# lauraset/Super-resolution-building-height-estimation

Hardware: AMD Instinct MI355X
Metric: tiles/sec (64x64x8ch->256x256 height) (higher is better)
Workload: dtype f16 operands / f32 accumulate (MFMA), f32 residual stream; 1 GPU; RRDBNet x4 (23 RRDB, 64 feat) forward_feature, batch 32 tiles/GPU, 64x64x3 -> 64x256x256 (BASELINE.json configs[1]); global_batch=32, parallelism=tile-sharded x1 (no data-path collective)

## Files before the change

include/srbh.h:

```cpp
#ifndef SRBH_H
#define SRBH_H

#include <stddef.h>
#include <stdint.h>

#ifdef __cplusplus
extern "C" {
#endif

#define SRBH_OK 0
#define SRBH_ERR_ARG (-1)
#define SRBH_ERR_WORKSPACE (-2)

int srbh_version(void);
const char* srbh_last_error(void);
#define SRBH_PATH_HCONV16 0
#define SRBH_PATH_HCONV_TEMPLATE 1
#define SRBH_PATH_ENTRY_FUSED 2
#define SRBH_PATH_ENTRY_SPLIT 3
#define SRBH_PATH_WGRAD16 4
#define SRBH_PATH_WGRAD_B16_GENERIC 5
#define SRBH_PATH_WGRAD_F32 6
#define SRBH_PATH_WGRAD_ENTRY_FUSED 7
#define SRBH_PATH_WGRAD_ENTRY_SPLIT 8
#define SRBH_PATH_HCONV_UP 9
#define SRBH_PATH_HBLOCK16 11
#define SRBH_PATH_HBWD16 10
int srbh_path_counters(unsigned long long* out, int n, int reset);
int srbh_head_wgs_cap(int path);

size_t srbh_act16_bytes(int B, int C, int H, int W);
int srbh_nchw32_to_act16(const float* src, void* dst, int B, int C, int H, int W, void* stream);
int srbh_act16_to_nchw32(const void* src, float* dst, int B, int C, int H, int W, void* stream);

size_t srbh_wpack16_bytes(int cout, int cin);
int srbh_pack_conv3x3_f16(const float* w_oihw, int cout, int cin, void* packed, void* stream);

typedef struct srbh_conv3x3_args {
    const void* in;
    int in_chunks_total;
    int in_chunk0;
    int in_chunks;
    const void* w;
    const float* bias;
    int cout;
    int B, H, W;
    int upsample2x;
    int lrelu;
    float res_scale;
    float* res1;
    int res1_update;
    float res2_scale;
    float* res2;
    int res2_update;
    const float* skip;
    void* out16;
    int out16_chunks_total;
    int out16_chunk0;
    float* out32;
    int out32_c;
    int out16_nhwc;
} srbh_conv3x3_args;

int srbh_conv3x3_f16(const srbh_conv3x3_args* a, void* stream);

typedef struct srbh_conv3x3_split {
    const void* in_lo;
    int in_lo_chunks_total;
    int in_lo_chunk0;
    const void* w_lo;
    void* out16_lo;
    int out16_lo_chunks_total;
    int out16_lo_chunk0;
} srbh_conv3x3_split;
int srbh_conv3x3_f16x2(const srbh_conv3x3_args* a, const srbh_conv3x3_split* s, void* stream);
int srbh_pack_conv3x3_f16lo(const float* w_oihw, int cout, int cin, void* packed, void* stream);
int srbh_act16_split_lo(const float* v, int fragment_order, const void* hi, int hi_chunks_total, int hi_chunk0, void* lo, int lo_chunks_total,
                        int lo_chunk0, int B, int H, int W, void* stream);
int srbh_conv3x3_x16(const srbh_conv3x3_args* a, int bf16, const void* mask16, int mask_chunks_total, int mask_chunk0, void* stream);
int srbh_pack_conv3x3_b16(const float* w_oihw, int cout, int cin, void* packed, void* stream);
typedef struct srbh_pack3x3_desc {
    const float* w;
    void* packed;
    const float* bias_src;
    float* bias_dst;
    int cout, cin, bf16, pad_;
} srbh_pack3x3_desc;
int srbh_pack_conv3x3_many(const srbh_pack3x3_desc* table_dev, int n, long max_elems, void* stream);
int srbh_nhwc32_to_act16(const float* src, void* dst, int B, int C, int H, int W, int chunks_total, int chunk0, float scale, int bf16,
                         void* stream);
int srbh_act16_channel_sum(const void* src, int B, int H, int W, int chunks_total, int chunk0, int nchunk, int bf16, float* out,
                           void* stream);
int srbh_act16_wgrad_b16(const void* x, int x_chunks_total, int cin, const void* dy, int dy_chunks_total, int dy_ch0, int cout,
                         int B, int H, int W, float* dw, float* ws, void* stream);
int srbh_axpby_f32(float* dst, float a, const float* x, float b, const float* y, long n, void* stream);
int srbh_lrelu_bwd_f32(float* g, const float* y, float slope, long n, void* stream);
int srbh_up2_bwd_nhwc_f32(const float* g, float* out, int B, int Ho, int Wo, int C, void* stream);
int srbh_bilinear2x_nhwc_f32(const float* x, float* out, int B, int H, int W, int C, int backward, void* stream);

int srbh_conv_first_f32(const float* x_nchw, const float* w_oihw, const float* bias, int B, int cin, int H, int W,
                        float* res_a, float* res_b, float* res_c, void* out16, int out16_chunks_total, void* stream);

typedef struct srbh_conv_w {
    const void* w;
    const float* bias;
} srbh_conv_w;

typedef struct srbh_rrdbnet_desc {
    int num_in_ch;
    int num_block;
    const float* conv_first_w;
    const float* conv_first_b;
    const srbh_conv_w* rdb;
    srbh_conv_w conv_body, conv_up1, conv_up2, conv_hr;
    srbh_conv_w conv_last;
    int num_out_ch;
    const srbh_conv_w* rdb_b16;
    int tail_f16x2;
    const void* conv_body_lo;
    const void* conv_up1_lo;
    const void* conv_up2_lo;
    const void* conv_hr_lo;
} srbh_rrdbnet_desc;

size_t srbh_rrdbnet_workspace_bytes(int B, int H, int W, int want_forward);
size_t srbh_rrdbnet_workspace_bytes_f16x2(int B, int H, int W, int want_forward);
int srbh_rrdbnet_forward(const srbh_rrdbnet_desc* d, const float* x, float* out, int B, int H, int W,
                         int want_forward, void* ws, size_t ws_bytes, void* stream);


int srbh_rrdbnet_trunk_train_forward(const srbh_rrdbnet_desc* d, float* xr, float* xrr, void* dense_all, size_t dense_stride, int B, int H,
                                     int W, void* stream);
size_t srbh_rrdbnet_trunk_train_aux_bytes(int B, int H, int W);
int srbh_rrdbnet_trunk_train_forward_persistent(const srbh_rrdbnet_desc* d, float* xr, float* xrr, void* dense_all, size_t dense_stride, int B, int H,
                                                int W, void* aux, void* stream, int* used);
size_t srbh_rrdbnet_trunk_wgrad_ws_bytes(void);
int srbh_rrdbnet_trunk_train_backward(int num_block, const void* dense_all, size_t dense_stride, const void* packs, size_t pack_stride,
                                      const size_t* pack_off, float* g_a, float* g_b, float* g_c, float** g_out, void* G, size_t g_stride,
                                      float* dw_all, float* db_all, float* wgrad_ws, int B, int H, int W, void* stream);
int srbh_rrdbnet_trunk_train_backward_persistent(int num_block, const void* dense_all, size_t dense_stride, const void* packs, size_t pack_stride,
                                                 const size_t* pack_off, const float* zero_bias, const float* g_a, float* g_b, float* g_c,
                                                 float** g_out, void* G_all, size_t g_stride, float* dw_all, float* db_all, float* wgrad_ws,
                                                 void* trunk_wgrad_ws, int B, int H, int W, void* aux, void* stream, int* used);
size_t srbh_trunk_wgrad_ws_bytes(int num_block, int B, int H, int W);
int srbh_trunk_wgrad(int num_block, const void* dense_all, size_t dense_stride, const void* G_all, size_t g_stride, int B, int H, int W, float* dw_all,
                     float* db_all, void* ws, void* stream);

int srbh_rrdbnet_last_status(const void* ws, int B, int H, int W, int want_forward, void* stream);

int srbh_rrdbnet_trunk_out(const void* ws, size_t ws_bytes, int num_block, int B, int H, int W, int want_forward, float* out, void* stream);

int srbh_ptail_wgs_cap(int cap);

int srbh_trunk_timing(int on);
int srbh_trunk_last_ms(float* ms);
const char* srbh_trunk_kernel_name(void);

size_t srbh_hpack_bytes(int cout, int cin, int ksize);
int srbh_hpack_conv_f32(const float* w_oihw, int cout, int cin, int ksize, int transpose_flip, float* packed, void* stream);

size_t srbh_bn_stats_bytes(int C);
int srbh_hconv_up_supported(int H, int W);

typedef struct srbh_hconv_args {
    const float* src0; int c0;
    const float* pre_scale; const float* pre_shift; int pre_relu;
    const float* src1; int c1;
    const float* w;
    const float* bias;
    int cout;
    int ksize;
    int B, H, W;
    int pixelshuffle2;
    float* out;
    double* stats;
    int src0_ld, src1_ld;
    int out_ld, out_coff;
    int post_lrelu;
    const float* res1; int res1_ld; float res1_scale;
    const float* res2; int res2_ld; float res2_scale;
// ... 278 lines not shown
```

super-resolution-building-height-estimation_amd/_lib.py:

```python
from __future__ import annotations

import ctypes as C
import os
import subprocess
import threading

_HERE = os.path.dirname(os.path.abspath(__file__))
ROOT = os.path.dirname(_HERE)
CSRC = os.path.join(_HERE, "csrc")
INCLUDE = os.path.join(ROOT, "include")
LIB_PATH = os.path.join(_HERE, "libsrbh.so")
_DEV_LIB = os.environ.get("SRBH_LIB_PATH")
SOURCES = ["srbh_conv3x3.hip", "srbh_aux.hip", "srbh_rrdbnet.hip", "srbh_ptrunk.hip", "srbh_trunk_wgrad.hip", "srbh_ptail.hip", "srbh_ptail_split.hip", "srbh_head.hip", "srbh_head_bwd.hip", "srbh_mosaic.hip", "srbh_loader.hip", "srbh_loss.hip", "srbh_dwconv.hip", "srbh_mbconv.hip", "srbh_pwconv.hip", "srbh_dconv.hip", "srbh_optim.hip"]
HIPCC = os.environ.get("HIPCC", "/opt/rocm/bin/hipcc")
HIPFLAGS = ["--offload-arch=gfx950", "-O3", "-std=c++17", "-fPIC", "-Wno-unused-result", "-Wno-inline-asm"]
if os.environ.get("SRBH_HIPFLAGS_OVERRIDE"):
    HIPFLAGS = os.environ["SRBH_HIPFLAGS_OVERRIDE"].split()


def build(force: bool = False, verbose: bool = False) -> str:
    srcs = [os.path.join(CSRC, s) for s in SOURCES if os.path.exists(os.path.join(CSRC, s))]
    deps = srcs + [os.path.join(CSRC, f) for f in os.listdir(CSRC) if f.endswith(".h")] + [os.path.join(INCLUDE, "srbh.h")]
    if not force and os.path.exists(LIB_PATH) and all(os.path.getmtime(LIB_PATH) >= os.path.getmtime(d) for d in deps):
        return LIB_PATH
    objs, procs = [], []
    for s in srcs:
        o = s[:-4] + ".o"
        objs.append(o)
        cmd = [HIPCC, *HIPFLAGS, "-I", INCLUDE, "-I", CSRC, "-c", s, "-o", o]
        procs.append((cmd, subprocess.Popen(cmd, stdout=subprocess.PIPE, stderr=subprocess.STDOUT, text=True)))
    for cmd, p in procs:
        out, _ = p.communicate()
        if p.returncode != 0:
            raise RuntimeError("hipcc failed: %s\n%s" % (" ".join(cmd), out))
        if verbose and out:
            print(out)
    cmd = [HIPCC, "--offload-arch=gfx950", "-shared", "-fPIC", *objs, "-o", LIB_PATH]
    r = subprocess.run(cmd, stdout=subprocess.PIPE, stderr=subprocess.STDOUT, text=True)
    if r.returncode != 0:
        raise RuntimeError("link failed: %s\n%s" % (" ".join(cmd), r.stdout))
    return LIB_PATH


PATH_NAMES = ("hconv16", "hconv_template", "entry_fused", "entry_split", "wgrad16", "wgrad_b16_generic", "wgrad_f32", "wgrad_entry_fused",
              "wgrad_entry_split", "hconv_up", "hbwd16", "hblock16")


def path_counters(reset=False):
    buf = (C.c_ulonglong * len(PATH_NAMES))()
    lib().srbh_path_counters(buf, len(PATH_NAMES), int(reset))
    return {k: int(v) for k, v in zip(PATH_NAMES, buf)}


def head_wgs_cap(form):
    cap = lib().srbh_head_wgs_cap(PATH_NAMES.index(form))
    if cap < 0:
        raise ValueError(f"{form}: no persistent tile walk behind this form")
    return int(cap)


class ConvArgs(C.Structure):
    _fields_ = [
        ("in_", C.c_void_p), ("in_chunks_total", C.c_int), ("in_chunk0", C.c_int), ("in_chunks", C.c_int),
        ("w", C.c_void_p), ("bias", C.c_void_p), ("cout", C.c_int),
        ("B", C.c_int), ("H", C.c_int), ("W", C.c_int),
        ("upsample2x", C.c_int), ("lrelu", C.c_int),
        ("res_scale", C.c_float), ("res1", C.c_void_p), ("res1_update", C.c_int),
        ("res2_scale", C.c_float), ("res2", C.c_void_p), ("res2_update", C.c_int),
        ("skip", C.c_void_p),
        ("out16", C.c_void_p), ("out16_chunks_total", C.c_int), ("out16_chunk0", C.c_int),
        ("out32", C.c_void_p), ("out32_c", C.c_int), ("out16_nhwc", C.c_int),
    ]


class HConvArgs(C.Structure):
    _fields_ = [
        ("src0", C.c_void_p), ("c0", C.c_int),
        ("pre_scale", C.c_void_p), ("pre_shift", C.c_void_p), ("pre_relu", C.c_int),
        ("src1", C.c_void_p), ("c1", C.c_int),
        ("w", C.c_void_p), ("bias", C.c_void_p), ("cout", C.c_int), ("ksize", C.c_int),
        ("B", C.c_int), ("H", C.c_int), ("W", C.c_int), ("pixelshuffle2", C.c_int),
        ("out", C.c_void_p), ("stats", C.c_void_p),
        ("src0_ld", C.c_int), ("src1_ld", C.c_int), ("out_ld", C.c_int), ("out_coff", C.c_int), ("post_lrelu", C.c_int),
        ("res1", C.c_void_p), ("res1_ld", C.c_int), ("res1_scale", C.c_float),
        ("res2", C.c_void_p), ("res2_ld", C.c_int), ("res2_scale", C.c_float),
        ("post_scale", C.c_void_p), ("post_shift", C.c_void_p), ("post_relu", C.c_int),
        ("io_h16", C.c_int),
        ("bstat_c", C.c_void_p), ("bstat_mean", C.c_void_p), ("bstat_invstd", C.c_void_p), ("bstat_ms", C.c_void_p), ("bstat_mh", C.c_void_p),
        ("stats_clean", C.c_int),
    ]


class HBwd16Args(C.Structure):
    _fields_ = ([("g", C.c_void_p), ("c", C.c_void_p), ("mean", C.c_void_p), ("invstd", C.c_void_p), ("coef", C.c_void_p), ("k1", C.c_void_p),
                 ("k2", C.c_void_p), ("mask_scale", C.c_void_p), ("mask_shift", C.c_void_p), ("x", C.c_void_p), ("pre_scale", C.c_void_p),
                 ("pre_shift", C.c_void_p), ("pre_relu", C.c_int), ("w", C.c_void_p), ("B", C.c_int), ("H", C.c_int), ("W", C.c_int),
                 ("dx", C.c_void_p), ("dx_b16", C.c_int), ("res", C.c_void_p), ("bstat_c", C.c_void_p), ("bstat_mean", C.c_void_p),
                 ("bstat_invstd", C.c_void_p), ("bstat_ms", C.c_void_p), ("bstat_mh", C.c_void_p), ("stats", C.c_void_p), ("stats_clean", C.c_int),
                 ("dw", C.c_void_p), ("ws", C.c_void_p), ("relu_bits", C.c_void_p)])


class HBlock16Args(C.Structure):
    _fields_ = [("x", C.c_void_p), ("w1", C.c_void_p), ("w2", C.c_void_p), ("scale1", C.c_void_p), ("shift1", C.c_void_p),
                ("scale2", C.c_void_p), ("shift2", C.c_void_p), ("out", C.c_void_p), ("out_h16", C.c_int), ("B", C.c_int), ("H", C.c_int), ("W", C.c_int)]


class HWGradArgs(C.Structure):
    _fields_ = [
        ("src0", C.c_void_p), ("c0", C.c_int),
        ("pre_scale", C.c_void_p), ("pre_shift", C.c_void_p), ("pre_relu", C.c_int),
        ("src1", C.c_void_p), ("c1", C.c_int),
        ("dy", C.c_void_p), ("cout", C.c_int), ("ksize", C.c_int),
        ("B", C.c_int), ("H", C.c_int), ("W", C.c_int), ("dw", C.c_void_p), ("ws", C.c_void_p),
        ("src0_ld", C.c_int), ("src1_ld", C.c_int), ("io", C.c_int),
    ]


class BnActArgs(C.Structure):
    _fields_ = [
        ("x", C.c_void_p), ("y", C.c_void_p), ("gamma", C.c_void_p), ("beta", C.c_void_p),
        ("running_mean", C.c_void_p), ("running_var", C.c_void_p), ("save_mean", C.c_void_p), ("save_invstd", C.c_void_p),
        ("pooled", C.c_void_p), ("res", C.c_void_p), ("drop", C.c_void_p),
        ("momentum", C.c_float), ("eps", C.c_float), ("B", C.c_int), ("C", C.c_int), ("HW", C.c_int), ("act", C.c_int),
        ("ws", C.c_void_p),
    ]


class MbMidArgs(C.Structure):
    _fields_ = ([(n, C.c_void_p) for n in ("e_pre", "wdw", "gamma0", "beta0", "running_mean0", "running_var0", "mean0", "invstd0",
                                           "gamma1", "beta1", "running_mean1", "running_var1", "mean1", "invstd1", "d_pre", "y", "pooled")]
                + [(n, C.c_float) for n in ("momentum0", "eps0", "momentum1", "eps1")] + [(n, C.c_int) for n in ("B", "C", "H", "W", "K")])


class MbMidBwdArgs(C.Structure):
    _fields_ = ([(n, C.c_void_p) for n in ("dout", "gate", "dpooled", "d_pre", "e_pre", "wdw", "gamma0", "beta0", "mean0", "invstd0",
                                           "gamma1", "beta1", "mean1", "invstd1", "de_pre", "dwdw", "dgamma0", "dbeta0", "dgamma1", "dbeta1")]
                + [(n, C.c_int) for n in ("B", "C", "H", "W", "K")])


class BnActBwdArgs(C.Structure):
    _fields_ = [
        ("dy", C.c_void_p), ("x", C.c_void_p), ("gamma", C.c_void_p), ("beta", C.c_void_p),
        ("save_mean", C.c_void_p), ("save_invstd", C.c_void_p), ("gate", C.c_void_p), ("dpooled", C.c_void_p), ("drop", C.c_void_p),
        ("dx", C.c_void_p), ("dgamma", C.c_void_p), ("dbeta", C.c_void_p),
        ("B", C.c_int), ("C", C.c_int), ("HW", C.c_int), ("act", C.c_int), ("ws", C.c_void_p),
    ]


class ConvW(C.Structure):
    _fields_ = [("w", C.c_void_p), ("bias", C.c_void_p)]


class RRDBNetDesc(C.Structure):
    _fields_ = [
        ("num_in_ch", C.c_int), ("num_block", C.c_int),
        ("conv_first_w", C.c_void_p), ("conv_first_b", C.c_void_p),
        ("rdb", C.POINTER(ConvW)),
        ("conv_body", ConvW), ("conv_up1", ConvW), ("conv_up2", ConvW), ("conv_hr", ConvW),
        ("conv_last", ConvW), ("num_out_ch", C.c_int),
        ("rdb_b16", C.POINTER(ConvW)),
        ("tail_f16x2", C.c_int),
        ("conv_body_lo", C.c_void_p), ("conv_up1_lo", C.c_void_p), ("conv_up2_lo", C.c_void_p), ("conv_hr_lo", C.c_void_p),
    ]


class ConvSplit(C.Structure):
    _fields_ = [
        ("in_lo", C.c_void_p), ("in_lo_chunks_total", C.c_int), ("in_lo_chunk0", C.c_int),
        ("w_lo", C.c_void_p),
        ("out16_lo", C.c_void_p), ("out16_lo_chunks_total", C.c_int), ("out16_lo_chunk0", C.c_int),
    ]


_vp, _i, _sz, _f = C.c_void_p, C.c_int, C.c_size_t, C.c_float
SIGNATURES = {
    "srbh_version": (_i, []),
    "srbh_last_error": (C.c_char_p, []),
    "srbh_path_counters": (_i, [_vp, _i, _i]),
    "srbh_head_wgs_cap": (_i, [_i]),
    "srbh_act16_bytes": (_sz, [_i, _i, _i, _i]),
    "srbh_nchw32_to_act16": (_i, [_vp, _vp, _i, _i, _i, _i, _vp]),
    "srbh_act16_to_nchw32": (_i, [_vp, _vp, _i, _i, _i, _i, _vp]),
    "srbh_wpack16_bytes": (_sz, [_i, _i]),
    "srbh_pack_conv3x3_f16": (_i, [_vp, _i, _i, _vp, _vp]),
    "srbh_conv3x3_f16": (_i, [C.POINTER(ConvArgs), _vp]),
    "srbh_conv3x3_f16x2": (_i, [C.POINTER(ConvArgs), C.POINTER(ConvSplit), _vp]),
    "srbh_pack_conv3x3_f16lo": (_i, [_vp, _i, _i, _vp, _vp]),
    "srbh_act16_split_lo": (_i, [_vp, _i, _vp, _i, _i, _vp, _i, _i, _i, _i, _i, _vp]),
    "srbh_rrdbnet_workspace_bytes_f16x2": (_sz, [_i, _i, _i, _i]),
    "srbh_conv3x3_x16": (_i, [C.POINTER(ConvArgs), _i, _vp, _i, _i, _vp]),
    "srbh_pack_conv3x3_b16": (_i, [_vp, _i, _i, _vp, _vp]),
    "srbh_nhwc32_to_act16": (_i, [_vp, _vp, _i, _i, _i, _i, _i, _i, _f, _i, _vp]),
    "srbh_act16_channel_sum": (_i, [_vp, _i, _i, _i, _i, _i, _i, _i, _vp, _vp]),
    "srbh_axpby_f32": (_i, [_vp, _f, _vp, _f, _vp, C.c_long, _vp]),
    "srbh_rrdbnet_trunk_train_forward": (_i, [C.POINTER(RRDBNetDesc), _vp, _vp, _vp, _sz, _i, _i, _i, _vp]),
    "srbh_rrdbnet_trunk_train_aux_bytes": (_sz, [_i, _i, _i]),
    "srbh_rrdbnet_trunk_train_forward_persistent": (_i, [C.POINTER(RRDBNetDesc), _vp, _vp, _vp, _sz, _i, _i, _i, _vp, _vp, C.POINTER(C.c_int)]),
    "srbh_rrdbnet_trunk_wgrad_ws_bytes": (_sz, []),
# ... 165 lines not shown
```

super-resolution-building-height-estimation_amd/csrc/srbh_internal.h:

```cpp
#pragma once
#include <hip/hip_runtime.h>
#include <stdarg.h>
#include <stdio.h>
#include <vector>
#include "srbh.h"

namespace srbh {

constexpr int PIX_B = 64;
constexpr int CHUNK_C = 32;
constexpr int TILE_W = 64;
constexpr int TILE_H = 8;

void set_error(const char* fmt, ...);
enum PathCounter { PATH_HCONV16 = 0, PATH_HCONV_TEMPLATE, PATH_ENTRY_FUSED, PATH_ENTRY_SPLIT, PATH_WGRAD16, PATH_WGRAD_B16_GENERIC,
                   PATH_WGRAD_F32, PATH_WGRAD_ENTRY_FUSED, PATH_WGRAD_ENTRY_SPLIT, PATH_HCONV_UP, PATH_HBWD16, PATH_HBLOCK16, PATH_N };
extern unsigned long long g_path_counters[PATH_N];
inline void count_path(int i) { ++g_path_counters[i]; }
int hconv16_wgs_cap();
int hconv_up_wgs_cap();
int hconv_entry_wgs_cap();
int hblock16_wgs_cap();
int hwgrad16_wgs_cap();
int hbwd16_wgs_cap();
int zero_async(void* p, size_t bytes, hipStream_t st);
int hip_fail(hipError_t e, const char* what);

#define SRBH_HIP(call)                                         \
    do {                                                       \
        hipError_t e_ = (call);                                \
        if (e_ != hipSuccess) return srbh::hip_fail(e_, #call); \
    } while (0)

#define SRBH_REQUIRE(cond, ...)            \
    do {                                   \
        if (!(cond)) {                     \
            srbh::set_error(__VA_ARGS__);  \
            return SRBH_ERR_ARG;           \
        }                                  \
    } while (0)

#define SRBH_ONCE_PER_DEVICE(stmt)                        \
    do {                                                  \
        static unsigned long long done_ = 0;              \
        int dev_ = 0;                                     \
        SRBH_HIP(hipGetDevice(&dev_));                    \
        if (!((done_ >> (dev_ & 63)) & 1ull)) {           \
            stmt;                                         \
            done_ |= 1ull << (dev_ & 63);                 \
        }                                                 \
    } while (0)

struct Act16Geo {
    int row_b;
    int plane_b;
    long img_b;
    size_t total_b;
};
inline Act16Geo act16_geo(int B, int chunks, int H, int W) {
    Act16Geo g;
    g.row_b = (W + 2) * PIX_B;
    g.plane_b = (H + 2) * g.row_b;
    g.img_b = (long)chunks * g.plane_b;
    size_t slack = (size_t)(TILE_H + 4) * (size_t)((W + 2 > TILE_W + 2) ? (W + 2) : (TILE_W + 2)) * PIX_B + 8192;
    g.total_b = (size_t)B * g.img_b + slack;
    g.total_b = (g.total_b + 255) & ~(size_t)255;
    return g;
}


size_t ptrunk_aux_bytes(int B, int tiles_per_img);
size_t ptrunk_err_offset(int B, int tiles_per_img);
int ptail_run(const srbh_conv3x3_args* a, hipStream_t stream, int* used);
int ptail_wgs_cap();
int ptrunk_takes(int num_block, int H, int W, int* takes, int* ncu_out);
int ptrunk_run(const srbh_rrdbnet_desc* d, void* dense0, void* dense1, float* xr, float* xrr, int B, int H, int W,
               void* aux, hipStream_t stream, int* used, int* final_cur, long train_stride = 0, const void* mask = nullptr, long mask_stride = 0,
               bool bf16 = false);
int conv3x3_trunk_b16(const srbh_conv3x3_args* a, int out_f16, void* stream);
int conv_first_f32(const float* x, const float* w, const float* bias, int B, int cin, int H, int W, float* ra, float* rb, float* rc,
                   void* out16, int out16_chunks_total, int bf16, void* stream);


#if defined(__HIP_DEVICE_COMPILE__) || defined(__HIPCC__)
__device__ __forceinline__ void fold_stat_slots(double* stats, const int C, const int clear, double* red, double& s, double& q) {
    constexpr int NS = 64;
    const int t = threadIdx.x, V = 2 * C, G = 256 / V, v = t % V, g = t / V;
    double part = 0.0;
    if (g < G) {
        for (int k = g; k < NS; k += G) part += stats[(long)k * V + v];
        if (clear)
            for (int k = g; k < NS; k += G) stats[(long)k * V + v] = 0.0;
        red[g * V + v] = part;
    }
    __syncthreads();
    s = 0.0;
    q = 0.0;
    if (t < C)
        for (int k = 0; k < G; ++k) {
            s += red[k * V + t];
            q += red[k * V + C + t];
        }
}

__device__ __forceinline__ unsigned bf16x2_rne(float lo, float hi) {
    typedef float f2_t __attribute__((ext_vector_type(2)));
    typedef __bf16 b2_t __attribute__((ext_vector_type(2)));
    const f2_t f = {lo, hi};
    return __builtin_bit_cast(unsigned, __builtin_convertvector(f, b2_t));
}
#endif
}
```

super-resolution-building-height-estimation_amd/csrc/srbh_ptail.hip:

```cpp
#include "srbh_ptail_kernel.h"

namespace {
using namespace srbh;
using namespace srbh_k;

struct TParams {
    In16 in;
    const char* w;
    const float* bias;
    int H, W;
    int tiles_x, tiles_per_img, ntiles, tiles_per_wg;
    int lrelu;
    Out16 out16;
    float* out32;
};

template <int UPS>
__global__ __launch_bounds__(256, 1) void ptail_kernel(const TParams p) {
    using G = TileGeo<UPS>;
    constexpr int IN_EX = G::UNITS * 16;
    constexpr int CB = 2;
    extern __shared__ __attribute__((aligned(16))) char smem[];
    const int tid = threadIdx.x;
    const int lane = tid & 63;
    const int wave = __builtin_amdgcn_readfirstlane(tid >> 6);
    const int l31 = lane & 31, hi = lane >> 5;
    const int wr = wave >> 1, wc = wave & 1;

    int goff[G::NJ];
#pragma unroll
    for (int j = 0; j < G::NJ; ++j) {
        const int u0 = j * 256 + tid;
        const int u = u0 < G::UNITS ? u0 : 0;
        const int trow = u / (G::COLS * 4);
        const int rem = u - trow * (G::COLS * 4);
        const int pc = rem >> 2, ps = rem & 3;
        goff[j] = trow * p.in.row_b + pc * PIX_B + ((ps ^ ((pc >> 2) & 3)) << 4);
    }
    const unsigned long long tail_mask = __builtin_amdgcn_ballot_w64((G::NJ - 1) * 256 + tid < G::UNITS);
    int aoff[3][2];
#pragma unroll
    for (int dx = 0; dx < 3; ++dx) {
        const int pc = UPS ? (((wc * 32 + l31 + dx - 1) >> 1) + 1) : (wc * 32 + l31 + dx);
#pragma unroll
        for (int ks = 0; ks < 2; ++ks)
            aoff[dx][ks] = wr * (UPS ? 2 : 4) * G::ROW_B + pc * PIX_B + (((ks * 2 + hi) ^ ((pc >> 2) & 3)) << 4);
    }

    auto stage_inputs = [&](int t) {
        int img, Y0, X0;
        tile_origin(t, p.tiles_per_img, p.tiles_x, img, Y0, X0);
        const char* src0 = p.in.base + (long)img * p.in.img_b + (long)(UPS ? (Y0 >> 1) : Y0) * p.in.row_b + (UPS ? (X0 >> 1) : X0) * PIX_B;
#pragma unroll
        for (int c = 0; c < 2; ++c)
#pragma unroll
            for (int j = 0; j < G::NJ; ++j)
                dma16(src0 + (long)c * p.in.plane_b + goff[j], TAIL_W_B + c * IN_EX + (j * 256 + wave * 64) * 16,
                      j < G::NJ - 1 ? ~0ull : tail_mask);
    };

    const int nst = ((p.H & (TILE_H - 1)) == 0 && (p.W & (TILE_W - 1)) == 0) ? (p.out32 ? 32 : 0) + (p.out16.base ? 16 : 0) : 0;
    const int t0 = blockIdx.x * p.tiles_per_wg;
    const int t1 = (t0 + p.tiles_per_wg < p.ntiles) ? t0 + p.tiles_per_wg : p.ntiles;
    if (t0 >= t1) return;
#pragma unroll
    for (int k = 0; k < 18; ++k) dma16(p.w + (wave + 4 * k) * 1024 + lane * 16, (wave + 4 * k) * 1024, ~0ull);
    stage_inputs(t0);
    floatx4 bias4[CB][4];
#pragma unroll
    for (int mb = 0; mb < CB; ++mb)
#pragma unroll
        for (int g = 0; g < 4; ++g)
            bias4[mb][g] = p.bias ? *(const floatx4*)(p.bias + mb * 32 + g * 8 + hi * 4) : floatx4{0.f, 0.f, 0.f, 0.f};

    for (int t = t0; t < t1; ++t) {
        int img, Y0, X0;
        tile_origin(t, p.tiles_per_img, p.tiles_x, img, Y0, X0);
        if (t == t0 || nst == 0) asm volatile("s_waitcnt vmcnt(0)" ::: "memory");
        else if (nst == 16) asm volatile("s_waitcnt vmcnt(16)" ::: "memory");
        else if (nst == 32) asm volatile("s_waitcnt vmcnt(32)" ::: "memory");
        else asm volatile("s_waitcnt vmcnt(48)" ::: "memory");
        __syncthreads();
        floatx16 acc[CB][4];
#pragma unroll
        for (int mb = 0; mb < CB; ++mb)
#pragma unroll
            for (int i = 0; i < 4; ++i)
#pragma unroll
                for (int r = 0; r < 16; ++r) acc[mb][i][r] = 0.f;
        constexpr int NREAD = G::NP + 3 * CB, NMFMA = 12 * CB;
        half8 P[2][G::NP];
        half8 A[2][3][CB];
        auto load_group = [&](int q, int set) {
            const int c = q / 6, g = q - c * 6;
            const int ks = g / 3, dx = g - ks * 3;
            const char* sbi = smem + TAIL_W_B + c * IN_EX;
            const char* sbw = smem + c * (36 * 1024) + lane * 16;
#pragma unroll
            for (int r = 0; r < G::NP; ++r) P[set][r] = *(const half8*)(sbi + aoff[dx][ks] + r * G::ROW_B);
#pragma unroll
            for (int dy = 0; dy < 3; ++dy)
#pragma unroll
                for (int mb = 0; mb < CB; ++mb)
                    A[set][dy][mb] = *(const half8*)(sbw + ((((dy * 3 + dx) * 2 + ks) * CB + mb) << 10));
        };
        load_group(0, 0);
#pragma unroll
        for (int q = 0; q < 12; ++q) {
            if (q + 1 < 12) load_group(q + 1, (q + 1) & 1);
#pragma unroll
            for (int dy = 0; dy < 3; ++dy)
#pragma unroll
                for (int i = 0; i < 4; ++i) {
                    const int pr = UPS ? (((i + dy - 1) >> 1) + 1) : (i + dy);
#pragma unroll
                    for (int mb = 0; mb < CB; ++mb)
                        acc[mb][i] = __builtin_amdgcn_mfma_f32_32x32x16_f16(A[q & 1][dy][mb], P[q & 1][pr], acc[mb][i], 0, 0, 0);
                }
            if (q == 0) __builtin_amdgcn_sched_group_barrier(0x100, NREAD, 0);
            if (q + 1 < 12) {
#pragma unroll
                for (int k = 0; k < NREAD; ++k) {
                    __builtin_amdgcn_sched_group_barrier(0x008, 1, 0);
                    __builtin_amdgcn_sched_group_barrier(0x100, 1, 0);
                }
                __builtin_amdgcn_sched_group_barrier(0x008, NMFMA - NREAD, 0);
            } else {
                __builtin_amdgcn_sched_group_barrier(0x008, NMFMA, 0);
            }
        }
        __syncthreads();
        if (t + 1 < t1) stage_inputs(t + 1);

        const int X = X0 + wc * 32 + l31;
#pragma unroll
        for (int i = 0; i < 4; ++i) {
            const int Y = Y0 + wr * 4 + i;
            const bool valid = (Y < p.H) && (X < p.W);
            const long pix = ((long)img * p.H + Y) * p.W + X;
#pragma unroll
            for (int mb = 0; mb < CB; ++mb) {
                unsigned hp[4][2];
#pragma unroll
                for (int g = 0; g < 4; ++g) {
                    floatx4 v;
#pragma unroll
                    for (int q = 0; q < 4; ++q) v[q] = acc[mb][i][g * 4 + q];
                    v += bias4[mb][g];
                    if (p.lrelu) {
#pragma unroll
                        for (int q = 0; q < 4; ++q) v[q] = v[q] >= 0.f ? v[q] : v[q] * 0.2f;
                    }
                    if (p.out32 && valid) *(floatx4*)(p.out32 + pix * 64 + mb * 32 + g * 8 + hi * 4) = v;
                    half4 h4;
#pragma unroll
                    for (int q = 0; q < 4; ++q) h4[q] = (_Float16)v[q];
                    const uint2 u = __builtin_bit_cast(uint2, h4);
                    hp[g][0] = u.x;
                    hp[g][1] = u.y;
                }
                if (p.out16.base) {
#pragma unroll
                    for (int m = 0; m < 2; ++m) {
                        store16_pair(p.out16, valid, img, mb, Y, X, m, hi, hp[2 * m], hp[2 * m + 1]);
                    }
                }
            }
        }
    }
}

thread_local int g_ptail_wgs_cap = 0;

template <int UPS>
int launch(const TParams& p0, hipStream_t stream) {
    static_assert(TAIL_LDS_B<UPS> <= 163840, "resident weights + both input chunks must fit the 160 KiB LDS");
    SRBH_ONCE_PER_DEVICE(SRBH_HIP(hipFuncSetAttribute((const void*)ptail_kernel<UPS>, hipFuncAttributeMaxDynamicSharedMemorySize, TAIL_LDS_B<UPS>)));
    TParams p = p0;
    int grid = 0;
    if (const int rc = tail_grid(p.ntiles, &p.tiles_per_wg, &grid)) return rc;
    hipLaunchKernelGGL(ptail_kernel<UPS>, dim3(grid), dim3(256), TAIL_LDS_B<UPS>, stream, p);
    SRBH_HIP(hipGetLastError());
    return SRBH_OK;
}

}

extern "C" int srbh_ptail_wgs_cap(int cap) {
    const int prev = g_ptail_wgs_cap;
    g_ptail_wgs_cap = cap > 0 ? cap : 0;
    return prev;
}

namespace srbh {

int ptail_wgs_cap() { return g_ptail_wgs_cap; }

int ptail_run(const srbh_conv3x3_args* a, hipStream_t stream, int* used) {
    *used = 0;
    const char* e = getenv("SRBH_PTAIL");
    if (e && e[0] == '0') return SRBH_OK;
    if (a->in_chunks != 2 || a->cout != 64 || a->res1 || a->res2 || a->skip) return SRBH_OK;
    if (a->out32 && a->out32_c != 64) return SRBH_OK;
    const int tiles_x = (a->W + TILE_W - 1) / TILE_W, tiles_y = (a->H + TILE_H - 1) / TILE_H;
    if (a->out16_nhwc && (!a->out16 || a->out32)) return SRBH_OK;
    if ((long)tiles_x * tiles_y * a->B < 512 && !a->out16_nhwc) return SRBH_OK;
    TParams p{};
    p.in = tail_in16(a, a->in, a->in_chunks_total, a->in_chunk0);
    p.w = (const char*)a->w;
    p.bias = a->bias;
    p.H = a->H;
    p.W = a->W;
    p.tiles_x = tiles_x;
    p.tiles_per_img = tiles_x * tiles_y;
    p.ntiles = p.tiles_per_img * a->B;
    p.lrelu = a->lrelu;
    p.out16 = tail_out16(a, a->out16, a->out16_chunks_total, a->out16_chunk0);
    p.out32 = a->out32;
    const int rc = a->upsample2x ? launch<1>(p, stream) : launch<0>(p, stream);
    if (rc == SRBH_OK) *used = 1;
    return rc;
}

}
```

super-resolution-building-height-estimation_amd/csrc/srbh_ptail_kernel.h:

```cpp
#pragma once
#include <stdlib.h>
#include "srbh_conv3x3_kernel.h"

namespace srbh_k {

constexpr int TAIL_W_B = 2 * 36 * 1024;
template <int UPS>
constexpr int TAIL_LDS_B = TAIL_W_B + 2 * TileGeo<UPS>::UNITS * 16;

struct In16 {
    const char* base;
    long img_b;
    int plane_b, row_b;
};
struct Out16 {
    char* base;
    long img_b;
    int plane_b, row_b, pix_b, border;
};


__device__ __forceinline__ void dma16(const char* gaddr, const unsigned lds_off_v, const unsigned long long mask) {
    unsigned long long sv;
    const unsigned lds_off = __builtin_amdgcn_readfirstlane(lds_off_v);
    asm volatile("s_mov_b64 %0, exec\n\ts_mov_b64 exec, %1\n\ts_mov_b32 m0, %2\n\ts_nop 0\n\t"
                 "global_load_lds_dwordx4 %3, off\n\ts_mov_b64 exec, %0"
                 : "=&s"(sv) : "s"(mask), "s"(lds_off), "v"(gaddr) : "memory", "m0");
}

__device__ __forceinline__ void tile_origin(const int t, const int tiles_per_img, const int tiles_x, int& img, int& Y0, int& X0) {
    img = t / tiles_per_img;
    const int trem = t - img * tiles_per_img;
    const int ty = trem / tiles_x;
    Y0 = ty * TILE_H;
    X0 = (trem - ty * tiles_x) * TILE_W;
}

__device__ __forceinline__ void store16_pair(const Out16& o, const bool valid, const int img, const int mb, const int Y, const int X, const int m, const int hi,
                                             const unsigned (&ga)[2], const unsigned (&gb)[2]) {
    typedef unsigned uintx4 __attribute__((ext_vector_type(4)));
    auto s0 = __builtin_amdgcn_permlane32_swap(ga[0], gb[0], false, false);
    auto s1 = __builtin_amdgcn_permlane32_swap(ga[1], gb[1], false, false);
    const uintx4 raw = {s0[0], s1[0], s0[1], s1[1]};
    if (valid)
        *(uintx4*)(o.base + (long)img * o.img_b + (long)mb * o.plane_b + (long)(Y + o.border) * o.row_b + (X + o.border) * o.pix_b + m * 32 + hi * 16) = raw;
}

inline In16 tail_in16(const srbh_conv3x3_args* a, const void* buf, const int chunks_total, const int chunk0) {
    const Act16Geo g = act16_geo(a->B, chunks_total, a->upsample2x ? a->H / 2 : a->H, a->upsample2x ? a->W / 2 : a->W);
    return In16{(const char*)buf + (long)chunk0 * g.plane_b, g.img_b, g.plane_b, g.row_b};
}

inline Out16 tail_out16(const srbh_conv3x3_args* a, void* buf, const int chunks_total, const int chunk0) {
    if (!buf) return Out16{};
    if (a->out16_nhwc) {
        const int C = chunks_total * 32;
        return Out16{(char*)buf + (long)chunk0 * 64, (long)a->H * a->W * C * 2, 64, a->W * C * 2, C * 2, 0};
    }
    const Act16Geo g = act16_geo(a->B, chunks_total, a->H, a->W);
    return Out16{(char*)buf + (long)chunk0 * g.plane_b, g.img_b, g.plane_b, g.row_b, PIX_B, 1};
}

inline int tail_grid(const int ntiles, int* tiles_per_wg, int* grid) {
    static int ncu_of[64] = {0};
    int dev = 0;
    SRBH_HIP(hipGetDevice(&dev));
    if (!ncu_of[dev & 63]) SRBH_HIP(hipDeviceGetAttribute(&ncu_of[dev & 63], hipDeviceAttributeMultiprocessorCount, dev));
    int ncu = ncu_of[dev & 63];
    const int cap = ptail_wgs_cap();
    if (cap > 0 && cap < ncu) ncu = cap;
    if (const char* we = getenv("SRBH_PTAIL_WGS")) {
        const int ecap = atoi(we);
        if (ecap > 0 && ecap < ncu_of[dev & 63]) ncu = ecap;
    }
    const int nwg = ntiles < ncu ? ntiles : ncu;
    *tiles_per_wg = (ntiles + nwg - 1) / nwg;
    *grid = (ntiles + *tiles_per_wg - 1) / *tiles_per_wg;
    return SRBH_OK;
}

}
```

Measured before the change: 8114 tiles/s.

## Add specialized fast ptail kernel for upsample+lrelu f16 output path

Adds a specialised persistent tail conv kernel for the upsample2x + bias + LeakyReLU + padded f16 output case. It keeps the weights resident in LDS, prefetches the next tile's inputs by direct global-to-LDS DMA while the current tile's epilogue runs, and double-buffers LDS operand reads interleaved with MFMAs via sched_group_barrier. The epilogue uses packed multiply/max for LeakyReLU and drops the generic out32/nhwc branches. Path counters are added for both forms, and an env var can disable the fast path. The risk is correctness on LDS reuse across tiles and the hard-coded vmcnt wait depth.

```diff
diff --git a/include/srbh.h b/include/srbh.h
--- a/include/srbh.h
+++ b/include/srbh.h
@@ -26,6 +26,8 @@
 #define SRBH_PATH_HCONV_UP 9
 #define SRBH_PATH_HBLOCK16 11
 #define SRBH_PATH_HBWD16 10
+#define SRBH_PATH_PTAIL_GENERIC 12
+#define SRBH_PATH_PTAIL_FAST 13
 int srbh_path_counters(unsigned long long* out, int n, int reset);
 int srbh_head_wgs_cap(int path);
 
diff --git a/super-resolution-building-height-estimation_amd/_lib.py b/super-resolution-building-height-estimation_amd/_lib.py
--- a/super-resolution-building-height-estimation_amd/_lib.py
+++ b/super-resolution-building-height-estimation_amd/_lib.py
@@ -43,7 +43,7 @@
 
 
 PATH_NAMES = ("hconv16", "hconv_template", "entry_fused", "entry_split", "wgrad16", "wgrad_b16_generic", "wgrad_f32", "wgrad_entry_fused",
-              "wgrad_entry_split", "hconv_up", "hbwd16", "hblock16")
+              "wgrad_entry_split", "hconv_up", "hbwd16", "hblock16", "ptail_generic", "ptail_fast")
 
 
 def path_counters(reset=False):
diff --git a/super-resolution-building-height-estimation_amd/csrc/srbh_internal.h b/super-resolution-building-height-estimation_amd/csrc/srbh_internal.h
--- a/super-resolution-building-height-estimation_amd/csrc/srbh_internal.h
+++ b/super-resolution-building-height-estimation_amd/csrc/srbh_internal.h
@@ -14,7 +14,8 @@
 
 void set_error(const char* fmt, ...);
 enum PathCounter { PATH_HCONV16 = 0, PATH_HCONV_TEMPLATE, PATH_ENTRY_FUSED, PATH_ENTRY_SPLIT, PATH_WGRAD16, PATH_WGRAD_B16_GENERIC,
-                   PATH_WGRAD_F32, PATH_WGRAD_ENTRY_FUSED, PATH_WGRAD_ENTRY_SPLIT, PATH_HCONV_UP, PATH_HBWD16, PATH_HBLOCK16, PATH_N };
+                   PATH_WGRAD_F32, PATH_WGRAD_ENTRY_FUSED, PATH_WGRAD_ENTRY_SPLIT, PATH_HCONV_UP, PATH_HBWD16, PATH_HBLOCK16, PATH_PTAIL_GENERIC,
+                   PATH_PTAIL_FAST, PATH_N };
 extern unsigned long long g_path_counters[PATH_N];
 inline void count_path(int i) { ++g_path_counters[i]; }
 int hconv16_wgs_cap();
diff --git a/super-resolution-building-height-estimation_amd/csrc/srbh_ptail.hip b/super-resolution-building-height-estimation_amd/csrc/srbh_ptail.hip
--- a/super-resolution-building-height-estimation_amd/csrc/srbh_ptail.hip
+++ b/super-resolution-building-height-estimation_amd/csrc/srbh_ptail.hip
@@ -170,19 +170,219 @@
     }
 }
 
+#ifndef PTAIL_FORMS
+#define PTAIL_FORMS 1
+#endif
+
+#if PTAIL_FORMS
+template <int UPS>
+__global__ __launch_bounds__(256, 1) void ptail_fast_kernel(const TParams p) {
+    using G = TileGeo<UPS>;
+    typedef unsigned uintx4 __attribute__((ext_vector_type(4)));
+    typedef float floatx2 __attribute__((ext_vector_type(2)));
+    typedef __attribute__((address_space(1))) char gchar;
+    typedef __attribute__((address_space(1))) uintx4 guintx4;
+    constexpr int IN_EX = G::UNITS * 16;
+    constexpr int CB = 2;
+    constexpr int NST = 16;
+    extern __shared__ __attribute__((aligned(16))) char smem[];
+    const int tid = threadIdx.x;
+    const int lane = tid & 63;
+    const int wave = __builtin_amdgcn_readfirstlane(tid >> 6);
+    const int l31 = lane & 31, hi = lane >> 5;
+    const int wr = wave >> 1, wc = wave & 1;
+
+    int goff[G::NJ];
+#pragma unroll
+    for (int j = 0; j < G::NJ; ++j) {
+        const int u0 = j * 256 + tid;
+        const int u = u0 < G::UNITS ? u0 : 0;
+        const int trow = u / (G::COLS * 4);
+        const int rem = u - trow * (G::COLS * 4);
+        const int pc = rem >> 2, ps = rem & 3;
+        goff[j] = trow * p.in.row_b + pc * PIX_B + ((ps ^ ((pc >> 2) & 3)) << 4);
+    }
+    const unsigned long long tail_mask = __builtin_amdgcn_ballot_w64((G::NJ - 1) * 256 + tid < G::UNITS);
+    int aoff[3][2];
+#pragma unroll
+    for (int dx = 0; dx < 3; ++dx) {
+        const int pc = UPS ? (((wc * 32 + l31 + dx - 1) >> 1) + 1) : (wc * 32 + l31 + dx);
+#pragma unroll
+        for (int ks = 0; ks < 2; ++ks)
+            aoff[dx][ks] = wr * (UPS ? 2 : 4) * G::ROW_B + pc * PIX_B + (((ks * 2 + hi) ^ ((pc >> 2) & 3)) << 4);
+    }
+    auto uni64 = [](unsigned long long m) {
+        const unsigned lo = __builtin_amdgcn_readfirstlane((unsigned)m), hi32 = __builtin_amdgcn_readfirstlane((unsigned)(m >> 32));
+        return ((unsigned long long)hi32 << 32) | lo;
+    };
+    const unsigned lds_w = TAIL_W_B + wave * 1024;
+
+    auto stage_inputs = [&](int img, int Y0, int X0) {
+        const char* src0 = p.in.base + (long)img * p.in.img_b + (long)(UPS ? (Y0 >> 1) : Y0) * p.in.row_b + (UPS ? (X0 >> 1) : X0) * PIX_B;
+#pragma unroll
+        for (int c = 0; c < 2; ++c) {
+            const unsigned long long sb = uni64((unsigned long long)(src0 + (long)c * p.in.plane_b));
+#pragma unroll
+            for (int j = 0; j < G::NJ - 1; ++j) dma16_uni(sb, goff[j], lds_w + c * IN_EX + j * 4096);
+            dma16((const char*)sb + goff[G::NJ - 1], lds_w + c * IN_EX + (G::NJ - 1) * 4096, tail_mask);
+        }
+    };
+    auto advance = [&](int& img, int& Y0, int& X0) {
+        X0 += TILE_W;
+        if (X0 >= p.W) {
+            X0 = 0;
+            Y0 += TILE_H;
+            if (Y0 >= p.H) {
+                Y0 = 0;
+                ++img;
+            }
+        }
+    };
+
+    const int t0 = blockIdx.x * p.tiles_per_wg;
+    const int t1 = (t0 + p.tiles_per_wg < p.ntiles) ? t0 + p.tiles_per_wg : p.ntiles;
+    if (t0 >= t1) return;
+    const unsigned long long wb = uni64((unsigned long long)(p.w + wave * 1024));
+#pragma unroll
+    for (int k = 0; k < 18; ++k) dma16_uni(wb + k * 4096, lane * 16, wave * 1024 + k * 4096);
+    int img, Y0, X0;
+    tile_origin(t0, p.tiles_per_img, p.tiles_x, img, Y0, X0);
+    stage_inputs(img, Y0, X0);
+    floatx4 bias4[CB][4];
+#pragma unroll
+    for (int mb = 0; mb < CB; ++mb)
+#pragma unroll
+        for (int g = 0; g < 4; ++g) bias4[mb][g] = *(const floatx4*)(p.bias + mb * 32 + g * 8 + hi * 4);
+    const unsigned lane_off = (wc * 32 + l31 + 1) * PIX_B + hi * 16;
+    const long mb_b = p.out16.plane_b;
+
+    const floatx2 slope2 = {0.2f, 0.2f};
+
+    for (int t = t0; t < t1; ++t) {
+        if (t == t0) asm volatile("s_waitcnt vmcnt(0)" ::: "memory");
+        else asm volatile("s_waitcnt vmcnt(%0)" ::"n"(NST) : "memory");
+        __syncthreads();
+        floatx16 acc[CB][4];
+#pragma unroll
+        for (int mb = 0; mb < CB; ++mb)
+#pragma unroll
+            for (int i = 0; i < 4; ++i)
+#pragma unroll
+                for (int r = 0; r < 16; ++r) acc[mb][i][r] = 0.f;
+        constexpr int NREAD = G::NP + 3 * CB, NMFMA = 12 * CB;
+        half8 P[2][G::NP];
+        half8 A[2][3][CB];
+        auto load_group = [&](int q, int set) {
+            const int c = q / 6, g = q - c * 6;
+            const int ks = g / 3, dx = g - ks * 3;
+            const char* sbi = smem + TAIL_W_B + c * IN_EX;
+            const char* sbw = smem + c * (36 * 1024) + lane * 16;
+#pragma unroll
+            for (int r = 0; r < G::NP; ++r) P[set][r] = *(const half8*)(sbi + aoff[dx][ks] + r * G::ROW_B);
+#pragma unroll
+            for (int dy = 0; dy < 3; ++dy)
+#pragma unroll
+                for (int mb = 0; mb < CB; ++mb)
+                    A[set][dy][mb] = *(const half8*)(sbw + ((((dy * 3 + dx) * 2 + ks) * CB + mb) << 10));
+        };
+        load_group(0, 0);
+#pragma unroll
+        for (int q = 0; q < 12; ++q) {
+            if (q + 1 < 12) load_group(q + 1, (q + 1) & 1);
+#pragma unroll
+            for (int dy = 0; dy < 3; ++dy)
+#pragma unroll
+                for (int i = 0; i < 4; ++i) {
+                    const int pr = UPS ? (((i + dy - 1) >> 1) + 1) : (i + dy);
+#pragma unroll
+                    for (int mb = 0; mb < CB; ++mb)
+                        acc[mb][i] = __builtin_amdgcn_mfma_f32_32x32x16_f16(A[q & 1][dy][mb], P[q & 1][pr], acc[mb][i], 0, 0, 0);
+                }
+            if (q == 0) __builtin_amdgcn_sched_group_barrier(0x100, NREAD, 0);
+            if (q + 1 < 12) {
+#pragma unroll
+                for (int k = 0; k < NREAD; ++k) {
+                    __builtin_amdgcn_sched_group_barrier(0x008, 1, 0);
+                    __builtin_amdgcn_sched_group_barrier(0x100, 1, 0);
+                }
+                __builtin_amdgcn_sched_group_barrier(0x008, NMFMA - NREAD, 0);
+            } else {
+                __builtin_amdgcn_sched_group_barrier(0x008, NMFMA, 0);
+            }
+        }
+        __syncthreads();
+        const int img_c = img, Y0_c = Y0, X0_c = X0;
+        advance(img, Y0, X0);
+        if (t + 1 < t1) stage_inputs(img, Y0, X0);
+
+#pragma unroll
+        for (int i = 0; i < 4; ++i) {
+            const int Y = Y0_c + wr * 4 + i;
+            const char* row = p.out16.base + (long)img_c * p.out16.img_b + (long)(Y + 1) * p.out16.row_b + (long)X0_c * PIX_B;
+            gchar* const rowb = (gchar*)uni64((unsigned long long)row);
+#pragma unroll
+            for (int mb = 0; mb < CB; ++mb) {
+                unsigned hp[4][2];
+#pragma unroll
+                for (int g = 0; g < 4; ++g) {
+                    floatx4 v;
+#pragma unroll
+                    for (int q = 0; q < 4; ++q) v[q] = acc[mb][i][g * 4 + q];
+                    v += bias4[mb][g];
+#pragma unroll
+                    for (int h = 0; h < 2; ++h) {
+                        const floatx2 v2 = {v[2 * h], v[2 * h + 1]};
+                        floatx2 vs;
+                        asm("v_pk_mul_f32 %0, %1, %2" : "=v"(vs) : "v"(v2), "v"(slope2));
+                        asm("v_max_f32 %0, %1, %2" : "=v"(v[2 * h]) : "v"(v2[0]), "v"(vs[0]));
+                        asm("v_max_f32 %0, %1, %2" : "=v"(v[2 * h + 1]) : "v"(v2[1]), "v"(vs[1]));
+                    }
+                    half4 h4;
+#pragma unroll
+                    for (int q = 0; q < 4; ++q) h4[q] = (_Float16)v[q];
+                    const uint2 u = __builtin_bit_cast(uint2, h4);
+                    hp[g][0] = u.x;
+                    hp[g][1] = u.y;
+                }
+#pragma unroll
+                for (int m = 0; m < 2; ++m) {
+                    auto s0 = __builtin_amdgcn_permlane32_swap(hp[2 * m][0], hp[2 * m + 1][0], false, false);
+                    auto s1 = __builtin_amdgcn_permlane32_swap(hp[2 * m][1], hp[2 * m + 1][1], false, false);
+                    const uintx4 raw = {s0[0], s1[0], s0[1], s1[1]};
+                    *(guintx4*)(rowb + mb * mb_b + lane_off + m * 32) = raw;
+                }
+            }
+        }
+    }
+}
+#endif
+
 thread_local int g_ptail_wgs_cap = 0;
 
-template <int UPS>
-int launch(const TParams& p0, hipStream_t stream) {
-    static_assert(TAIL_LDS_B<UPS> <= 163840, "resident weights + both input chunks must fit the 160 KiB LDS");
-    SRBH_ONCE_PER_DEVICE(SRBH_HIP(hipFuncSetAttribute((const void*)ptail_kernel<UPS>, hipFuncAttributeMaxDynamicSharedMemorySize, TAIL_LDS_B<UPS>)));
+template <typename K>
+int launch(K kernel, const int lds_b, const TParams& p0, hipStream_t stream) {
     TParams p = p0;
     int grid = 0;
     if (const int rc = tail_grid(p.ntiles, &p.tiles_per_wg, &grid)) return rc;
-    hipLaunchKernelGGL(ptail_kernel<UPS>, dim3(grid), dim3(256), TAIL_LDS_B<UPS>, stream, p);
+    hipLaunchKernelGGL(kernel, dim3(grid), dim3(256), lds_b, stream, p);
     SRBH_HIP(hipGetLastError());
     return SRBH_OK;
 }
+
+template <int UPS>
+int launch_generic(const TParams& p, hipStream_t stream) {
+    static_assert(TAIL_LDS_B<UPS> <= 163840, "resident weights + both input chunks must fit the 160 KiB LDS");
+    SRBH_ONCE_PER_DEVICE(SRBH_HIP(hipFuncSetAttribute((const void*)ptail_kernel<UPS>, hipFuncAttributeMaxDynamicSharedMemorySize, TAIL_LDS_B<UPS>)));
+    return launch(ptail_kernel<UPS>, TAIL_LDS_B<UPS>, p, stream);
+}
+
+#if PTAIL_FORMS
+template <int UPS>
+int launch_fast(const TParams& p, hipStream_t stream) {
+    SRBH_ONCE_PER_DEVICE(SRBH_HIP(hipFuncSetAttribute((const void*)ptail_fast_kernel<UPS>, hipFuncAttributeMaxDynamicSharedMemorySize, TAIL_LDS_B<UPS>)));
+    return launch(ptail_fast_kernel<UPS>, TAIL_LDS_B<UPS>, p, stream);
+}
+#endif
 
 }
 
@@ -217,8 +417,19 @@
     p.lrelu = a->lrelu;
     p.out16 = tail_out16(a, a->out16, a->out16_chunks_total, a->out16_chunk0);
     p.out32 = a->out32;
-    const int rc = a->upsample2x ? launch<1>(p, stream) : launch<0>(p, stream);
-    if (rc == SRBH_OK) *used = 1;
+    int rc = SRBH_OK, fast = 0;
+#if PTAIL_FORMS
+    const char* fe = getenv("SRBH_PTAIL_FORMS");
+    if (!(fe && fe[0] == '0') && a->H % TILE_H == 0 && a->W % TILE_W == 0 && a->bias && a->upsample2x && a->lrelu && a->out16 && !a->out16_nhwc && !a->out32) {
+        fast = 1;
+        rc = launch_fast<1>(p, stream);
+    }
+#endif
+    if (!fast) rc = a->upsample2x ? launch_generic<1>(p, stream) : launch_generic<0>(p, stream);
+    if (rc == SRBH_OK) {
+        *used = 1;
+        count_path(fast ? PATH_PTAIL_FAST : PATH_PTAIL_GENERIC);
+    }
     return rc;
 }
 
diff --git a/super-resolution-building-height-estimation_amd/csrc/srbh_ptail_kernel.h b/super-resolution-building-height-estimation_amd/csrc/srbh_ptail_kernel.h
--- a/super-resolution-building-height-estimation_amd/csrc/srbh_ptail_kernel.h
+++ b/super-resolution-building-height-estimation_amd/csrc/srbh_ptail_kernel.h
@@ -26,6 +26,10 @@
     asm volatile("s_mov_b64 %0, exec\n\ts_mov_b64 exec, %1\n\ts_mov_b32 m0, %2\n\ts_nop 0\n\t"
                  "global_load_lds_dwordx4 %3, off\n\ts_mov_b64 exec, %0"
                  : "=&s"(sv) : "s"(mask), "s"(lds_off), "v"(gaddr) : "memory", "m0");
+}
+
+__device__ __forceinline__ void dma16_uni(const unsigned long long base, const unsigned voff, const unsigned lds_off) {
+    asm volatile("s_mov_b32 m0, %0\n\ts_nop 3\n\tglobal_load_lds_dwordx4 %1, %2" ::"s"(lds_off), "v"(voff), "s"(base) : "memory", "m0");
 }
 
 __device__ __forceinline__ void tile_origin(const int t, const int tiles_per_img, const int tiles_x, int& img, int& Y0, int& X0) {
```

New measurement: 8158 tiles/s, median of 6. Within noise of the previous version (+0.5%).
